# yoshitomo-matsubara/sc2-benchmark

Hardware: AMD Instinct MI355X
Metric: images/s + bpp, Entropic-Student ResNet-50 224^2 (higher is better)
Workload: dtype bf16

## Files before the change

### sc2-benchmark_amd/csrc/conv1x1_pair.hip

```cpp
#include <stdlib.h>

#include <atomic>

#include "gfx950_prims.h"

#ifndef SC2_NT_PAIR
#define SC2_NT_PAIR 0
#endif

namespace {

using namespace sc2prim;

#ifndef SC2_PAIR_DBG
#define SC2_PAIR_DBG 0
#endif

struct PairArgs {
    const uint16_t *__restrict__ o;
    const uint16_t *__restrict__ w3;
    const float *__restrict__ b3;
    const uint16_t *__restrict__ idn;
    uint16_t *__restrict__ h;
    const uint16_t *__restrict__ w1;
    const float *__restrict__ b1;
    uint16_t *__restrict__ u;
    int M, n_tiles;
    int rev;
    unsigned *tile_ctr;
};

template <int C, int K1, int N2, int MT>
__global__ __launch_bounds__(512, 2) void conv1x1_pair_kernel(const PairArgs p) {
    constexpr int P = MT * 16;
    constexpr int KS1 = K1 / 32, KS2 = C / 32;
    constexpr int NT1 = C / 8 / 16;
    constexpr int ROWB = C * 2;
    constexpr int CPR = ROWB / 16;
    constexpr int IMG = P * ROWB, SLAB = P * 64, OT = KS1 * SLAB;
    constexpr int NT2 = N2 / 128;
    static_assert(N2 == 128 || N2 == 256, "one or two 16-channel tiles of u per wave");
    static_assert(N2 <= C, "the u staging lives in the image region");
    static_assert(CPR == 64, "one image row = one LDS-DMA wave-instruction");
    constexpr int UROW = N2 * 2, UCPR = UROW / 16;
    constexpr int OQ = (P * K1 * 2 / 16 + 511) / 512;
    constexpr int UQ = (P * UCPR + 511) / 512;
    constexpr int IQ = (P * CPR + 511) / 512;
    extern __shared__ __attribute__((aligned(16))) unsigned char smem[];
    unsigned char *img = smem;
    unsigned char *ot = smem + IMG;
    volatile int *next_slot = reinterpret_cast<volatile int *>(smem + IMG + OT);
    float *bias_lds = reinterpret_cast<float *>(smem + IMG + OT + 16);

    const uint32_t lds_base = (uint32_t)(uintptr_t)(lds_ptr_t)smem;
    const int tid = threadIdx.x, lane = tid & 63;
    const int wn = __builtin_amdgcn_readfirstlane(tid >> 6);

    constexpr uint32_t OOB = 0x80000000u;
    const buf_rsrc_t rs_idn = make_rsrc(p.idn, (uint32_t)((long long)p.M * ROWB));
    const buf_rsrc_t rs_o = make_rsrc(p.o, (uint32_t)((long long)p.M * K1 * 2));
    const buf_rsrc_t rs_h = make_rsrc(p.h, (uint32_t)((long long)p.M * ROWB));
    const buf_rsrc_t rs_u = make_rsrc(p.u, (uint32_t)((long long)p.M * N2 * 2));

    auto load_o = [&](int tile, uint4 (&ov)[OQ], int tq) {
        const bool t_ok = tile < p.n_tiles;
        const int tpos = p.rev ? p.n_tiles - 1 - tile : tile;
        const uint32_t so = (uint32_t)(t_ok ? (long long)tpos * P * (K1 * 2) : 0);
#pragma unroll
        for (int k = 0; k < OQ; ++k) {
            const int q = tq + 512 * k;
            const bool ok = t_ok && q < P * (K1 / 8) && (long long)tpos * P + q / (K1 / 8) < p.M;
            ov[k] = buf_load16(rs_o, ok ? (uint32_t)q * 16u : OOB, so);
        }
    };
    auto store_o = [&](const uint4 (&ov)[OQ], int tq) {
#pragma unroll
        for (int k = 0; k < OQ; ++k) {
            const int q = tq + 512 * k;
            if (q < P * (K1 / 8)) {
                const int row = q / (K1 / 8), c16 = q % (K1 / 8);
                lds_write16(lds_base + IMG + (c16 >> 2) * SLAB + row * 64 + (((c16 & 3) ^ ((row >> 1) & 3)) << 4),
                            __builtin_bit_cast(u32x4_t, ov[k]));
            }
        }
    };
    auto issue_identity = [&](int tile, int lq) {
        static_assert(P % 8 == 0, "every wave takes P / 8 rows: straight-line issue, exact vmcnt bookkeeping");
#pragma unroll
        for (int r = 0; r < P / 8; ++r) {
            const int row = wn + 8 * r;
            const long long m = (long long)(p.rev ? p.n_tiles - 1 - tile : tile) * P + row;
            const bool ok = tile < p.n_tiles && m < p.M && !(SC2_PAIR_DBG & 1);
            const uint32_t voff = ok ? (uint32_t)((lq ^ (row & 15)) << 4) : OOB;
            buf_load_lds16(rs_idn, (lds_ptr_t)(img + row * ROWB), voff, (uint32_t)(ok ? m * ROWB : 0));
        }
    };

    uint4 wv[KS1][NT1];
    const buf_rsrc_t rs_w3 = make_rsrc(p.w3, (uint32_t)(C * K1 * 2));
    const uint32_t w3_vo = (uint32_t)(((wn * NT1) * KS1 * 64 + lane) * 16);
    auto load_w = [&]() {
#pragma unroll
        for (int j = 0; j < NT1; ++j)
#pragma unroll
            for (int s = 0; s < KS1; ++s) wv[s][j] = buf_load16(rs_w3, w3_vo, (uint32_t)((j * KS1 + s) * 1024));
    };
    load_w();
    const buf_rsrc_t rs_w1 = make_rsrc(p.w1, (uint32_t)(N2 * C * 2));
    const uint32_t w1_vo = (uint32_t)(((wn * NT2) * KS2 * 64 + lane) * 16);

    for (int k = tid; k < C + N2; k += 512) bias_lds[k] = k < C ? p.b3[k] : p.b1[k - C];
    int tile = blockIdx.x;
    int next_tile = tile + gridDim.x;
    {
        uint4 ov[OQ];
        load_o(tile, ov, tid);
        store_o(ov, tid);
        issue_identity(tile, lane);
    }
    __syncthreads();

    bool first = true;
    while (tile < p.n_tiles) {
        const long long m0 = (long long)(p.rev ? p.n_tiles - 1 - tile : tile) * P;
        int tq = tid, lq = lane;
        asm volatile("" : "+v"(tq), "+v"(lq));
        const int frow = lq & 15, fq = lq >> 4;
        const int o_lane = frow * 64 + ((fq ^ ((frow >> 1) & 3)) << 4);
        const int img_row = frow * ROWB;
        unsigned claimed = 0;
        if (tid == 0) {
            const unsigned one = 1u;
            asm volatile("global_atomic_add %0, %1, %2, off sc0" : "=v"(claimed) : "v"(p.tile_ctr), "v"(one) : "memory");
        }
        f32x4_t acc[MT][NT1];
#pragma unroll
        for (int i = 0; i < MT; ++i)
#pragma unroll
            for (int j = 0; j < NT1; ++j) acc[i][j] = f32x4_t{0.f, 0.f, 0.f, 0.f};
        {
            const uint32_t o_addr = lds_base + IMG + o_lane;
#pragma unroll
            for (int s = 0; s < KS1; ++s) {
                u32x4_t xa[4], xb[3];
                static_assert(MT == 7, "the asm waits below name 4 + 3 registers");
                xa[0] = lds_read16_imm<0 * 1024>(o_addr + s * SLAB);
                xa[1] = lds_read16_imm<1 * 1024>(o_addr + s * SLAB);
                xa[2] = lds_read16_imm<2 * 1024>(o_addr + s * SLAB);
                xa[3] = lds_read16_imm<3 * 1024>(o_addr + s * SLAB);
                asm volatile("s_waitcnt lgkmcnt(0)" : "+v"(xa[0]), "+v"(xa[1]), "+v"(xa[2]), "+v"(xa[3])::"memory");
                xb[0] = lds_read16_imm<4 * 1024>(o_addr + s * SLAB);
                xb[1] = lds_read16_imm<5 * 1024>(o_addr + s * SLAB);
                xb[2] = lds_read16_imm<6 * 1024>(o_addr + s * SLAB);
#pragma unroll
                for (int i = 0; i < 4; ++i) {
                    const bf16x8_t xf = __builtin_bit_cast(bf16x8_t, xa[i]);
#pragma unroll
                    for (int j = 0; j < NT1; ++j)
                        acc[i][j] = __builtin_amdgcn_mfma_f32_16x16x32_bf16(__builtin_bit_cast(bf16x8_t, wv[s][j]), xf, acc[i][j], 0, 0, 0);
                }
                asm volatile("s_waitcnt lgkmcnt(0)" : "+v"(xb[0]), "+v"(xb[1]), "+v"(xb[2])::"memory");
#pragma unroll
                for (int i = 0; i < 3; ++i) {
                    const bf16x8_t xf = __builtin_bit_cast(bf16x8_t, xb[i]);
#pragma unroll
                    for (int j = 0; j < NT1; ++j)
                        acc[4 + i][j] = __builtin_amdgcn_mfma_f32_16x16x32_bf16(__builtin_bit_cast(bf16x8_t, wv[s][j]), xf, acc[4 + i][j], 0, 0, 0);
                }
                __builtin_amdgcn_sched_barrier(0);
            }
        }
        if (first) asm volatile("s_waitcnt vmcnt(0)" ::: "memory");
        else if (wn == 0) asm volatile("s_waitcnt vmcnt(%0)" ::"n"(IQ + UQ + 1) : "memory");
        else asm volatile("s_waitcnt vmcnt(%0)" ::"n"(IQ + UQ) : "memory");
        first = false;
        __syncthreads();
#pragma unroll
        for (int j = 0; j < NT1; ++j) {
            const int c16 = wn * (NT1 * 2) + j * 2 + (fq >> 1);
            const float4 b3v = *reinterpret_cast<const float4 *>(bias_lds + wn * (NT1 * 16) + j * 16 + fq * 4);
            const f32x2_t b01 = {b3v.x, b3v.y}, b23 = {b3v.z, b3v.w};
            const int slot_lane = img_row + ((c16 ^ frow) << 4) + (fq & 1) * 8;
#pragma unroll
            for (int i = 0; i < MT; ++i) {
                unsigned char *slot = img + slot_lane + i * (16 * ROWB);
                const uint2 xr = *reinterpret_cast<const uint2 *>(slot);
                f32x2_t v01 = f32x2_t{acc[i][j][0], acc[i][j][1]} + b01;
                f32x2_t v23 = f32x2_t{acc[i][j][2], acc[i][j][3]} + b23;
                v01 += f32x2_t{__builtin_bit_cast(float, xr.x << 16), __builtin_bit_cast(float, xr.x & 0xFFFF0000u)};
                v23 += f32x2_t{__builtin_bit_cast(float, xr.y << 16), __builtin_bit_cast(float, xr.y & 0xFFFF0000u)};
                v01 = f32x2_t{fmaxf(v01[0], 0.f), fmaxf(v01[1], 0.f)};
                v23 = f32x2_t{fmaxf(v23[0], 0.f), fmaxf(v23[1], 0.f)};
                uint2 o2;
                o2.x = pack2(v01);
                o2.y = pack2(v23);
                *reinterpret_cast<uint2 *>(slot) = o2;
                if ((i & 3) == 3) __builtin_amdgcn_sched_barrier(0);
            }
        }
        __syncthreads();
        __builtin_amdgcn_sched_barrier(0);
        constexpr int GB = 8;
        uint4 gb[GB][NT2];
#pragma unroll
        for (int ks = 0; ks < GB; ++ks)
#pragma unroll
            for (int t = 0; t < NT2; ++t) gb[ks][t] = buf_load16(rs_w1, w1_vo, (uint32_t)((t * KS2 + ks) * 1024));
        uint4 ov[OQ];
        load_o(next_tile, ov, tq);
        f32x4_t acc2[MT][NT2];
#pragma unroll
        for (int i = 0; i < MT; ++i)
#pragma unroll
            for (int t = 0; t < NT2; ++t) acc2[i][t] = f32x4_t{0.f, 0.f, 0.f, 0.f};
#pragma unroll
        for (int ks = 0; ks < ((SC2_PAIR_DBG & 4) ? 0 : KS2); ++ks) {
            bf16x8_t gf[NT2];
#pragma unroll
            for (int t = 0; t < NT2; ++t) {
                gf[t] = __builtin_bit_cast(bf16x8_t, gb[ks % GB][t]);
                if (ks + GB < KS2) gb[ks % GB][t] = buf_load16(rs_w1, w1_vo, (uint32_t)((t * KS2 + ks + GB) * 1024));
            }
            const int rd_lane = img_row + (((ks * 4 + fq) ^ frow) << 4);
#pragma unroll
            for (int i = 0; i < MT; ++i) {
                const bf16x8_t xf = __builtin_bit_cast(bf16x8_t, *reinterpret_cast<const uint4 *>(img + rd_lane + i * (16 * ROWB)));
#pragma unroll
                for (int t = 0; t < NT2; ++t) acc2[i][t] = __builtin_amdgcn_mfma_f32_16x16x32_bf16(gf[t], xf, acc2[i][t], 0, 0, 0);
            }
            if ((ks & 1) == 1) __builtin_amdgcn_sched_barrier(0);
        }
        if (tid == 0) {
            asm volatile("s_waitcnt vmcnt(%1)" : "+v"(claimed) : "n"(OQ) : "memory");
            *next_slot = (int)(claimed + 2 * gridDim.x);
            if (claimed == (unsigned)(p.n_tiles - 1)) *p.tile_ctr = 0u;
        }
        u32x4_t hv[IQ];
#pragma unroll
        for (int k = 0; k < IQ; ++k) {
            const int q = tq + 512 * k;
            const int row = q / CPR, c = q % CPR;
            hv[k] = *reinterpret_cast<const u32x4_t *>(img + row * ROWB + ((c ^ (row & 15)) << 4));
        }
        __syncthreads();
        store_o(ov, tq);
#pragma unroll
        for (int t = 0; t < NT2; ++t) {
            const float4 b1v = *reinterpret_cast<const float4 *>(bias_lds + C + (wn * NT2 + t) * 16 + fq * 4);
            const f32x2_t b01 = {b1v.x, b1v.y}, b23 = {b1v.z, b1v.w};
            const int c16 = (wn * NT2 + t) * 2 + (fq >> 1);
            const int u_lane = frow * UROW + ((c16 ^ frow) << 4) + (fq & 1) * 8;
#pragma unroll
            for (int i = 0; i < MT; ++i) {
                f32x2_t v01 = f32x2_t{acc2[i][t][0], acc2[i][t][1]} + b01;
                f32x2_t v23 = f32x2_t{acc2[i][t][2], acc2[i][t][3]} + b23;
                v01 = f32x2_t{fmaxf(v01[0], 0.f), fmaxf(v01[1], 0.f)};
                v23 = f32x2_t{fmaxf(v23[0], 0.f), fmaxf(v23[1], 0.f)};
                uint2 o2;
                o2.x = pack2(v01);
                o2.y = pack2(v23);
                *reinterpret_cast<uint2 *>(img + u_lane + i * (16 * UROW)) = o2;
            }
        }
        asm volatile("s_waitcnt lgkmcnt(0)" ::: "memory");
        __syncthreads();
        const int tile_after_next = __builtin_amdgcn_readfirstlane(*next_slot);
        u32x4_t uv[UQ];
#pragma unroll
        for (int k = 0; k < UQ; ++k) {
            const int q = tq + 512 * k;
            const int row = q / UCPR, c = q % UCPR;
            const int qq = q < P * UCPR ? row * UROW + ((c ^ (row & 15)) << 4) : 0;
            uv[k] = *reinterpret_cast<const u32x4_t *>(img + qq);
        }
        __syncthreads();
        issue_identity(next_tile, lq);
        {
            const uint32_t so = (uint32_t)(m0 * ROWB);
#pragma unroll
            for (int k = 0; k < IQ; ++k) {
                const int q = tq + 512 * k;
                buf_store16<SC2_NT_PAIR>(rs_h, (q < P * CPR && m0 + q / CPR < p.M && !(SC2_PAIR_DBG & 2)) ? (uint32_t)q * 16u : OOB, so, hv[k]);
            }
        }
        {
            const uint32_t so = (uint32_t)(m0 * UROW);
#pragma unroll
            for (int k = 0; k < UQ; ++k) {
                const int q = tq + 512 * k;
                buf_store16<SC2_NT_PAIR>(rs_u, (q < P * UCPR && m0 + q / UCPR < p.M && !(SC2_PAIR_DBG & 2)) ? (uint32_t)q * 16u : OOB, so, uv[k]);
            }
        }
        tile = next_tile;
        next_tile = tile_after_next;
    }
}

constexpr int kRing = 256;
sc2_counter_ring g_ring;
std::atomic<unsigned> g_seq{0};

template <int C, int K1, int N2, int MT>
int launch_pair(const PairArgs &a, hipStream_t s) {
    constexpr int P = MT * 16;
    constexpr int lds = P * C * 2 + (K1 / 32) * P * 64 + 16 + (C + N2) * 4;
    static_assert(lds <= 160 * 1024, "image + o tile must fit the CU's LDS");
    static bool attr_set[SC2_MAX_DEVICES] = {};
    const int dev = sc2_device_slot();
    if (!attr_set[dev]) {
        (void)hipFuncSetAttribute(reinterpret_cast<const void *>(&conv1x1_pair_kernel<C, K1, N2, MT>),
                                  hipFuncAttributeMaxDynamicSharedMemorySize, lds);
        attr_set[dev] = true;
    }
    const int g_cus = sc2_device_cus();
    unsigned *slot = g_ring.launch_slot(s, kRing, 1, g_seq);
    if (!slot) return SC2_ERR_INTERNAL;
    PairArgs b = a;
    b.n_tiles = (a.M + P - 1) / P;
    b.tile_ctr = slot;
    {
        const int alt = sc2_pol().pair_alt;
        static std::atomic<unsigned> calls{0};
        b.rev = alt ? (int)(calls.fetch_add(1) & 1u) : 0;
    }
    const int grid = b.n_tiles < g_cus ? b.n_tiles : g_cus;
    hipLaunchKernelGGL((conv1x1_pair_kernel<C, K1, N2, MT>), dim3(grid), dim3(512), lds, s, b);
    SC2_CHECK_LAUNCH();
    return SC2_OK;
}

}

extern "C" int sc2_conv1x1_pair_supported(int K1, int C, int N2) { return (K1 == 128 && C == 512 && (N2 == 128 || N2 == 256)) ? 1 : 0; }

extern "C" int sc2_conv1x1_pair_fwd(const void *o, const void *w3_frag, const float *b3, const void *identity, void *h,
                                    const void *w1_frag, const float *b1, void *u, long long M, int K1, int C, int N2,
                                    void *stream) {
    SC2_REQUIRE(o && w3_frag && b3 && identity && h && w1_frag && b1 && u, SC2_ERR_INVALID_ARG, "conv1x1_pair: null argument");
    SC2_REQUIRE(sc2_conv1x1_pair_supported(K1, C, N2), SC2_ERR_UNSUPPORTED, "conv1x1_pair: K1 %d C %d N2 %d not supported", K1, C, N2);
    SC2_REQUIRE(M > 0 && M * C * 2 < 0x7FF00000LL, SC2_ERR_UNSUPPORTED, "conv1x1_pair: M = %lld outside the 32-bit buffer range", M);
    PairArgs a;
    a.o = static_cast<const uint16_t *>(o); a.w3 = static_cast<const uint16_t *>(w3_frag); a.b3 = b3;
    a.idn = static_cast<const uint16_t *>(identity); a.h = static_cast<uint16_t *>(h);
    a.w1 = static_cast<const uint16_t *>(w1_frag); a.b1 = b1; a.u = static_cast<uint16_t *>(u);
    a.M = (int)M; a.n_tiles = 0; a.tile_ctr = nullptr; a.rev = 0;
    if (N2 == 256) return launch_pair<512, 128, 256, 7>(a, static_cast<hipStream_t>(stream));
    return launch_pair<512, 128, 128, 7>(a, static_cast<hipStream_t>(stream));
}
```

Baseline: 45720.

## Add double-buffered identity image pair kernel with register-resident W1 for N2=128

Adds a second fused conv1x1 pair kernel that keeps two image buffers in LDS, so the identity tile for the tile after next streams in while the current tile is computed. W1 is held in registers beside W3, which removes the per-tile W1 reloads, and the row tile shrinks from 7 to 3 MMA row tiles. The N2=128 path now dispatches to this kernel by default. It also adds optional memtime stamp instrumentation behind a compile flag. Smaller tiles mean more tiles and more atomic claims, and register pressure rises.

```diff
diff --git a/sc2-benchmark_amd/csrc/conv1x1_pair.hip b/sc2-benchmark_amd/csrc/conv1x1_pair.hip
--- a/sc2-benchmark_amd/csrc/conv1x1_pair.hip
+++ b/sc2-benchmark_amd/csrc/conv1x1_pair.hip
@@ -14,6 +14,33 @@
 
 #ifndef SC2_PAIR_DBG
 #define SC2_PAIR_DBG 0
+#endif
+
+#ifndef SC2_PAIR_STAMPS
+#define SC2_PAIR_STAMPS 0
+#endif
+constexpr int N_STAMP = 12;
+#if SC2_PAIR_STAMPS
+#include <stdio.h>
+#define PAIR_STAMPS_BEGIN unsigned long long st_sum[N_STAMP] = {}, st_last = __builtin_amdgcn_s_memtime(); const unsigned long long st_first = st_last
+#define PAIR_STAMP(k)                                                   \
+    do {                                                                \
+        __builtin_amdgcn_sched_barrier(0);                              \
+        const unsigned long long t_ = __builtin_amdgcn_s_memtime();     \
+        st_sum[k] += t_ - st_last;                                      \
+        st_last = t_;                                                   \
+        __builtin_amdgcn_sched_barrier(0);                              \
+    } while (0)
+#define PAIR_STAMPS_END                                                                                        \
+    do {                                                                                                       \
+        st_sum[10] = st_last - st_first;                                                                       \
+        if (p.stamps && lane == 0)                                                                             \
+            for (int k = 0; k < N_STAMP; ++k) p.stamps[((size_t)blockIdx.x * 8 + wn) * N_STAMP + k] = st_sum[k]; \
+    } while (0)
+#else
+#define PAIR_STAMPS_BEGIN do {} while (0)
+#define PAIR_STAMP(k) do {} while (0)
+#define PAIR_STAMPS_END do {} while (0)
 #endif
 
 struct PairArgs {
@@ -28,6 +55,9 @@
     int M, n_tiles;
     int rev;
     unsigned *tile_ctr;
+#if SC2_PAIR_STAMPS
+    unsigned long long *stamps;
+#endif
 };
 
 template <int C, int K1, int N2, int MT>
@@ -121,6 +151,7 @@
     __syncthreads();
 
     bool first = true;
+    PAIR_STAMPS_BEGIN;
     while (tile < p.n_tiles) {
         const long long m0 = (long long)(p.rev ? p.n_tiles - 1 - tile : tile) * P;
         int tq = tid, lq = lane;
@@ -170,11 +201,14 @@
                 __builtin_amdgcn_sched_barrier(0);
             }
         }
+        PAIR_STAMP(0);
         if (first) asm volatile("s_waitcnt vmcnt(0)" ::: "memory");
         else if (wn == 0) asm volatile("s_waitcnt vmcnt(%0)" ::"n"(IQ + UQ + 1) : "memory");
         else asm volatile("s_waitcnt vmcnt(%0)" ::"n"(IQ + UQ) : "memory");
         first = false;
+        PAIR_STAMP(1);
         __syncthreads();
+        PAIR_STAMP(2);
 #pragma unroll
         for (int j = 0; j < NT1; ++j) {
             const int c16 = wn * (NT1 * 2) + j * 2 + (fq >> 1);
@@ -199,6 +233,7 @@
             }
         }
         __syncthreads();
+        PAIR_STAMP(3);
         __builtin_amdgcn_sched_barrier(0);
         constexpr int GB = 8;
         uint4 gb[GB][NT2];
@@ -230,6 +265,7 @@
             }
             if ((ks & 1) == 1) __builtin_amdgcn_sched_barrier(0);
         }
+        PAIR_STAMP(4);
         if (tid == 0) {
             asm volatile("s_waitcnt vmcnt(%1)" : "+v"(claimed) : "n"(OQ) : "memory");
             *next_slot = (int)(claimed + 2 * gridDim.x);
@@ -243,6 +279,7 @@
             hv[k] = *reinterpret_cast<const u32x4_t *>(img + row * ROWB + ((c ^ (row & 15)) << 4));
         }
         __syncthreads();
+        PAIR_STAMP(5);
         store_o(ov, tq);
 #pragma unroll
         for (int t = 0; t < NT2; ++t) {
@@ -264,6 +301,7 @@
         }
         asm volatile("s_waitcnt lgkmcnt(0)" ::: "memory");
         __syncthreads();
+        PAIR_STAMP(6);
         const int tile_after_next = __builtin_amdgcn_readfirstlane(*next_slot);
         u32x4_t uv[UQ];
 #pragma unroll
@@ -274,6 +312,7 @@
             uv[k] = *reinterpret_cast<const u32x4_t *>(img + qq);
         }
         __syncthreads();
+        PAIR_STAMP(7);
         issue_identity(next_tile, lq);
         {
             const uint32_t so = (uint32_t)(m0 * ROWB);
@@ -293,7 +332,341 @@
         }
         tile = next_tile;
         next_tile = tile_after_next;
-    }
+        PAIR_STAMP(8);
+#if SC2_PAIR_STAMPS
+        st_sum[11] += 1;
+#endif
+    }
+    PAIR_STAMPS_END;
+}
+
+template <int OFF>
+__device__ __forceinline__ u32x2_t lds_read8_imm(uint32_t addr) {
+    u32x2_t v;
+    asm volatile("ds_read_b64 %0, %1 offset:%2" : "=v"(v) : "v"(addr), "n"(OFF) : "memory");
+    return v;
+}
+template <int OFF>
+__device__ __forceinline__ void lds_write8_imm(uint32_t addr, u32x2_t v) {
+    asm volatile("ds_write_b64 %0, %1 offset:%2" ::"v"(addr), "v"(v), "n"(OFF) : "memory");
+}
+__device__ __forceinline__ void wg_barrier() { asm volatile("s_waitcnt lgkmcnt(0)\n\ts_barrier" ::: "memory"); }
+
+template <int C, int K1, int N2, int MT>
+__global__ __launch_bounds__(512, 2) void conv1x1_pair_2img_kernel(const PairArgs p) {
+    constexpr int P = MT * 16;
+    constexpr int KS1 = K1 / 32, KS2 = C / 32;
+    constexpr int NT1 = C / 8 / 16;
+    constexpr int ROWB = C * 2;
+    constexpr int CPR = ROWB / 16;
+    constexpr int OQ = (P * K1 * 2 / 16 + 511) / 512;
+    constexpr int PO = OQ * 512 / (K1 / 8);
+    static_assert(PO >= P && OQ * 512 % (K1 / 8) == 0, "whole padded rows");
+    constexpr int IMG = P * ROWB, SLAB = PO * 64, OT = KS1 * SLAB;
+    constexpr int NT2 = N2 / 128;
+    static_assert(NT2 == 1, "W1 resident in registers beside W3 (64 + 64); N2 = 256 would take 128 and stays on the kernel above");
+    static_assert(N2 <= C, "the u staging lives in the image region");
+    static_assert(CPR == 64, "one image row = one LDS-DMA wave-instruction");
+    static_assert(P % 8 == 0, "every wave takes P / 8 identity rows: straight-line issue, exact vmcnt bookkeeping");
+    static_assert((MT - 1) * 16 * ROWB < 65536, "row tiles are reached through the 16-bit offset field");
+    constexpr int UROW = N2 * 2, UCPR = UROW / 16;
+    constexpr int UQ = (P * UCPR + 511) / 512;
+    constexpr int IQ = (P * CPR + 511) / 512;
+    static_assert(P * CPR == IQ * 512, "every thread reads IQ whole chunks of the image");
+    constexpr int SLOT = 2 * IMG + OT, BIAS = SLOT + 16;
+    extern __shared__ __attribute__((aligned(16))) unsigned char smem[];
+
+    const uint32_t lds_base = (uint32_t)(uintptr_t)(lds_ptr_t)smem;
+    const int tid = threadIdx.x, lane = tid & 63;
+    const int wn = __builtin_amdgcn_readfirstlane(tid >> 6);
+
+    constexpr uint32_t OOB = 0x80000000u;
+    const buf_rsrc_t rs_idn = make_rsrc(p.idn, (uint32_t)((long long)p.M * ROWB));
+    const buf_rsrc_t rs_o = make_rsrc(p.o, (uint32_t)((long long)p.M * K1 * 2));
+    const buf_rsrc_t rs_h = make_rsrc(p.h, (uint32_t)((long long)p.M * ROWB));
+    const buf_rsrc_t rs_u = make_rsrc(p.u, (uint32_t)((long long)p.M * N2 * 2));
+
+    auto load_o = [&](int tile, uint4 (&ov)[OQ], int tq) {
+        const bool t_ok = tile < p.n_tiles;
+        const int tpos = p.rev ? p.n_tiles - 1 - tile : tile;
+        const uint32_t so = (uint32_t)(t_ok ? (long long)tpos * P * (K1 * 2) : 0);
+#pragma unroll
+        for (int k = 0; k < OQ; ++k) {
+            const int q = tq + 512 * k;
+            const bool ok = t_ok && q < P * (K1 / 8) && (long long)tpos * P + q / (K1 / 8) < p.M;
+            ov[k] = buf_load16(rs_o, ok ? (uint32_t)q * 16u : OOB, so);
+        }
+    };
+    auto store_o = [&](const uint4 (&ov)[OQ], int tq) {
+#pragma unroll
+        for (int k = 0; k < OQ; ++k) {
+            const int q = tq + 512 * k;
+            const int row = q / (K1 / 8), c16 = q % (K1 / 8);
+            lds_write16(lds_base + 2 * IMG + (c16 >> 2) * SLAB + row * 64 + (((c16 & 3) ^ ((row >> 1) & 3)) << 4),
+                        __builtin_bit_cast(u32x4_t, ov[k]));
+        }
+    };
+    auto issue_identity = [&](int tile, uint32_t buf, int lq) {
+#pragma unroll
+        for (int r = 0; r < P / 8; ++r) {
+            const int row = wn + 8 * r;
+            const long long m = (long long)(p.rev ? p.n_tiles - 1 - tile : tile) * P + row;
+            const bool ok = tile < p.n_tiles && m < p.M && !(SC2_PAIR_DBG & 1);
+            const uint32_t voff = ok ? (uint32_t)((lq ^ (row & 15)) << 4) : OOB;
+            buf_load_lds16(rs_idn, (lds_ptr_t)(smem + buf + row * ROWB), voff, (uint32_t)(ok ? m * ROWB : 0));
+        }
+    };
+
+    {
+        float *bias_lds = reinterpret_cast<float *>(smem + BIAS);
+        for (int k = tid; k < C + N2; k += 512) bias_lds[k] = k < C ? p.b3[k] : p.b1[k - C];
+    }
+    int tile = blockIdx.x;
+    int next_tile = tile + gridDim.x;
+    issue_identity(tile, 0, lane);
+    issue_identity(next_tile, IMG, lane);
+    u32x4_t wv[KS1][NT1];
+    const buf_rsrc_t rs_w3 = make_rsrc(p.w3, (uint32_t)(C * K1 * 2));
+    const uint32_t w3_vo = (uint32_t)(((wn * NT1) * KS1 * 64 + lane) * 16);
+#pragma unroll
+    for (int j = 0; j < NT1; ++j)
+#pragma unroll
+        for (int s = 0; s < KS1; ++s) wv[s][j] = __builtin_bit_cast(u32x4_t, buf_load16(rs_w3, w3_vo, (uint32_t)((j * KS1 + s) * 1024)));
+    const buf_rsrc_t rs_w1 = make_rsrc(p.w1, (uint32_t)(N2 * C * 2));
+    const uint32_t w1_vo = (uint32_t)(((wn * NT2) * KS2 * 64 + lane) * 16);
+    u32x4_t w1v[KS2];
+#pragma unroll
+    for (int ks = 0; ks < KS2; ++ks) w1v[ks] = __builtin_bit_cast(u32x4_t, buf_load16(rs_w1, w1_vo, (uint32_t)(ks * 1024)));
+    {
+        uint4 ov[OQ];
+        load_o(tile, ov, tid);
+        store_o(ov, tid);
+    }
+#pragma unroll
+    for (int j = 0; j < NT1; ++j)
+#pragma unroll
+        for (int s = 0; s < KS1; ++s) asm volatile("" : "+v"(wv[s][j]));
+#pragma unroll
+    for (int ks = 0; ks < KS2; ++ks) asm volatile("" : "+v"(w1v[ks]));
+    asm volatile("s_waitcnt vmcnt(0)" ::: "memory");
+    wg_barrier();
+
+    uint32_t cur = 0;
+    PAIR_STAMPS_BEGIN;
+    while (tile < p.n_tiles) {
+        const long long m0 = (long long)(p.rev ? p.n_tiles - 1 - tile : tile) * P;
+        int tq = tid, lq = lane;
+        asm volatile("" : "+v"(tq), "+v"(lq));
+        const int frow = lq & 15, fq = lq >> 4;
+        const uint32_t o_addr = lds_base + 2 * IMG + frow * 64 + ((fq ^ ((frow >> 1) & 3)) << 4);
+        const uint32_t img_cur = lds_base + cur;
+        const uint32_t img_row = img_cur + frow * ROWB;
+        unsigned claimed = 0;
+        if (tid == 0) {
+            const unsigned one = 1u;
+            asm volatile("global_atomic_add %0, %1, %2, off sc0" : "=v"(claimed) : "v"(p.tile_ctr), "v"(one) : "memory");
+        }
+        f32x4_t acc[MT][NT1];
+#pragma unroll
+        for (int i = 0; i < MT; ++i)
+#pragma unroll
+            for (int j = 0; j < NT1; ++j) acc[i][j] = f32x4_t{0.f, 0.f, 0.f, 0.f};
+        static_assert(MT == 3, "the asm waits below name three registers per k-step");
+        {
+            u32x4_t x[2][MT];
+            x[0][0] = lds_read16_imm<0 * 1024>(o_addr);
+            x[0][1] = lds_read16_imm<1 * 1024>(o_addr);
+            x[0][2] = lds_read16_imm<2 * 1024>(o_addr);
+#pragma unroll
+            for (int s = 0; s < KS1; ++s) {
+                u32x4_t(&xc)[MT] = x[s & 1];
+                if (s + 1 < KS1) {
+                    u32x4_t(&xn)[MT] = x[(s + 1) & 1];
+                    xn[0] = lds_read16_imm<0 * 1024>(o_addr + (s + 1) * SLAB);
+                    xn[1] = lds_read16_imm<1 * 1024>(o_addr + (s + 1) * SLAB);
+                    xn[2] = lds_read16_imm<2 * 1024>(o_addr + (s + 1) * SLAB);
+                    asm volatile("s_waitcnt lgkmcnt(%3)" : "+v"(xc[0]), "+v"(xc[1]), "+v"(xc[2]) : "n"(MT) : "memory");
+                } else {
+                    asm volatile("s_waitcnt lgkmcnt(0)" : "+v"(xc[0]), "+v"(xc[1]), "+v"(xc[2])::"memory");
+                }
+#pragma unroll
+                for (int i = 0; i < MT; ++i) {
+                    const bf16x8_t xf = __builtin_bit_cast(bf16x8_t, xc[i]);
+#pragma unroll
+                    for (int j = 0; j < NT1; ++j)
+                        acc[i][j] = __builtin_amdgcn_mfma_f32_16x16x32_bf16(__builtin_bit_cast(bf16x8_t, wv[s][j]), xf, acc[i][j], 0, 0, 0);
+                }
+                __builtin_amdgcn_sched_barrier(0);
+            }
+        }
+        PAIR_STAMP(0);
+        u32x4_t b3r[NT1];
+#pragma unroll
+        for (int j = 0; j < NT1; ++j) b3r[j] = lds_read16_imm<0>(lds_base + (uint32_t)(BIAS + (wn * (NT1 * 16) + j * 16 + fq * 4) * 4));
+        if (wn == 0) asm volatile("s_waitcnt vmcnt(%0)" ::"n"(P / 8 + IQ + UQ + 1) : "memory");
+        else asm volatile("s_waitcnt vmcnt(%0)" ::"n"(P / 8 + IQ + UQ) : "memory");
+        PAIR_STAMP(1);
+        wg_barrier();
+        PAIR_STAMP(2);
+        {
+            u32x2_t xr[NT1][MT];
+            uint32_t slot[NT1];
+#pragma unroll
+            for (int j = 0; j < NT1; ++j) {
+                const int c16 = wn * (NT1 * 2) + j * 2 + (fq >> 1);
+                slot[j] = img_row + ((c16 ^ frow) << 4) + (fq & 1) * 8;
+                xr[j][0] = lds_read8_imm<0 * 16 * ROWB>(slot[j]);
+                xr[j][1] = lds_read8_imm<1 * 16 * ROWB>(slot[j]);
+                xr[j][2] = lds_read8_imm<2 * 16 * ROWB>(slot[j]);
+            }
+#pragma unroll
+            for (int j = 0; j < NT1; ++j) {
+                asm volatile("s_waitcnt lgkmcnt(%4)" : "+v"(xr[j][0]), "+v"(xr[j][1]), "+v"(xr[j][2]), "+v"(b3r[j]) : "n"(MT * (NT1 - 1)) : "memory");
+                const f32x4_t b3v = __builtin_bit_cast(f32x4_t, b3r[j]);
+                const f32x2_t b01 = {b3v[0], b3v[1]}, b23 = {b3v[2], b3v[3]};
+                u32x2_t o2[MT];
+#pragma unroll
+                for (int i = 0; i < MT; ++i) {
+                    f32x2_t v01 = f32x2_t{acc[i][j][0], acc[i][j][1]} + b01;
+                    f32x2_t v23 = f32x2_t{acc[i][j][2], acc[i][j][3]} + b23;
+                    v01 += f32x2_t{bf_lo(xr[j][i][0]), bf_hi(xr[j][i][0])};
+                    v23 += f32x2_t{bf_lo(xr[j][i][1]), bf_hi(xr[j][i][1])};
+                    v01 = f32x2_t{fmaxf(v01[0], 0.f), fmaxf(v01[1], 0.f)};
+                    v23 = f32x2_t{fmaxf(v23[0], 0.f), fmaxf(v23[1], 0.f)};
+                    o2[i] = u32x2_t{pack2(v01), pack2(v23)};
+                }
+                lds_write8_imm<0 * 16 * ROWB>(slot[j], o2[0]);
+                lds_write8_imm<1 * 16 * ROWB>(slot[j], o2[1]);
+                lds_write8_imm<2 * 16 * ROWB>(slot[j], o2[2]);
+            }
+        }
+        wg_barrier();
+        PAIR_STAMP(3);
+        __builtin_amdgcn_sched_barrier(0);
+        uint4 ov[OQ];
+        load_o(next_tile, ov, tq);
+        f32x4_t acc2[MT][NT2];
+#pragma unroll
+        for (int i = 0; i < MT; ++i)
+#pragma unroll
+            for (int t = 0; t < NT2; ++t) acc2[i][t] = f32x4_t{0.f, 0.f, 0.f, 0.f};
+        {
+            constexpr int KS2E = (SC2_PAIR_DBG & 4) ? 0 : KS2;
+            u32x4_t x[2][MT];
+            {
+                const uint32_t a = img_row + ((fq ^ frow) << 4);
+                x[0][0] = lds_read16_imm<0 * 16 * ROWB>(a);
+                x[0][1] = lds_read16_imm<1 * 16 * ROWB>(a);
+                x[0][2] = lds_read16_imm<2 * 16 * ROWB>(a);
+            }
+#pragma unroll
+            for (int ks = 0; ks < KS2E; ++ks) {
+                u32x4_t(&xc)[MT] = x[ks & 1];
+                if (ks + 1 < KS2E) {
+                    u32x4_t(&xn)[MT] = x[(ks + 1) & 1];
+                    const uint32_t a = img_row + ((((ks + 1) * 4 + fq) ^ frow) << 4);
+                    xn[0] = lds_read16_imm<0 * 16 * ROWB>(a);
+                    xn[1] = lds_read16_imm<1 * 16 * ROWB>(a);
+                    xn[2] = lds_read16_imm<2 * 16 * ROWB>(a);
+                    asm volatile("s_waitcnt lgkmcnt(%3)" : "+v"(xc[0]), "+v"(xc[1]), "+v"(xc[2]) : "n"(MT) : "memory");
+                } else {
+                    asm volatile("s_waitcnt lgkmcnt(0)" : "+v"(xc[0]), "+v"(xc[1]), "+v"(xc[2])::"memory");
+                }
+                const bf16x8_t gf = __builtin_bit_cast(bf16x8_t, w1v[ks]);
+#pragma unroll
+                for (int i = 0; i < MT; ++i)
+                    acc2[i][0] = __builtin_amdgcn_mfma_f32_16x16x32_bf16(gf, __builtin_bit_cast(bf16x8_t, xc[i]), acc2[i][0], 0, 0, 0);
+                if ((ks & 1) == 1) __builtin_amdgcn_sched_barrier(0);
+            }
+            if (KS2E == 0) asm volatile("s_waitcnt lgkmcnt(0)" : "+v"(x[0][0]), "+v"(x[0][1]), "+v"(x[0][2])::"memory");
+        }
+        PAIR_STAMP(4);
+        if (tid == 0) {
+            asm volatile("s_waitcnt vmcnt(%1)" : "+v"(claimed) : "n"(OQ) : "memory");
+            const unsigned nxt = claimed + 2 * gridDim.x;
+            asm volatile("ds_write_b32 %0, %1" ::"v"(lds_base + (uint32_t)SLOT), "v"(nxt) : "memory");
+            if (claimed == (unsigned)(p.n_tiles - 1)) *p.tile_ctr = 0u;
+        }
+        u32x4_t hv[IQ];
+#pragma unroll
+        for (int k = 0; k < IQ; ++k) {
+            const int q = tq + 512 * k;
+            const int row = q / CPR, c = q % CPR;
+            hv[k] = __builtin_bit_cast(u32x4_t, lds_read16(img_cur + row * ROWB + ((c ^ (row & 15)) << 4)));
+        }
+        static_assert(IQ == 6, "the wait below names six registers");
+        asm volatile("s_waitcnt lgkmcnt(0)" : "+v"(hv[0]), "+v"(hv[1]), "+v"(hv[2]), "+v"(hv[3]), "+v"(hv[4]), "+v"(hv[5])::"memory");
+        wg_barrier();
+        PAIR_STAMP(5);
+        store_o(ov, tq);
+        {
+            u32x4_t b1r[NT2];
+#pragma unroll
+            for (int t = 0; t < NT2; ++t) b1r[t] = lds_read16_imm<0>(lds_base + (uint32_t)(BIAS + C * 4 + ((wn * NT2 + t) * 16 + fq * 4) * 4));
+            asm volatile("s_waitcnt lgkmcnt(0)" : "+v"(b1r[0])::"memory");
+#pragma unroll
+            for (int t = 0; t < NT2; ++t) {
+                const f32x4_t b1v = __builtin_bit_cast(f32x4_t, b1r[t]);
+                const f32x2_t b01 = {b1v[0], b1v[1]}, b23 = {b1v[2], b1v[3]};
+                const int c16 = (wn * NT2 + t) * 2 + (fq >> 1);
+                const uint32_t u_lane = img_cur + frow * UROW + ((c16 ^ frow) << 4) + (fq & 1) * 8;
+                u32x2_t o2[MT];
+#pragma unroll
+                for (int i = 0; i < MT; ++i) {
+                    f32x2_t v01 = f32x2_t{acc2[i][t][0], acc2[i][t][1]} + b01;
+                    f32x2_t v23 = f32x2_t{acc2[i][t][2], acc2[i][t][3]} + b23;
+                    v01 = f32x2_t{fmaxf(v01[0], 0.f), fmaxf(v01[1], 0.f)};
+                    v23 = f32x2_t{fmaxf(v23[0], 0.f), fmaxf(v23[1], 0.f)};
+                    o2[i] = u32x2_t{pack2(v01), pack2(v23)};
+                }
+                lds_write8_imm<0 * 16 * UROW>(u_lane, o2[0]);
+                lds_write8_imm<1 * 16 * UROW>(u_lane, o2[1]);
+                lds_write8_imm<2 * 16 * UROW>(u_lane, o2[2]);
+            }
+        }
+        wg_barrier();
+        PAIR_STAMP(6);
+        unsigned slot_v;
+        asm volatile("ds_read_b32 %0, %1" : "=v"(slot_v) : "v"(lds_base + (uint32_t)SLOT) : "memory");
+        u32x4_t uv[UQ];
+#pragma unroll
+        for (int k = 0; k < UQ; ++k) {
+            const int q = tq + 512 * k;
+            const int row = q / UCPR, c = q % UCPR;
+            const int qq = q < P * UCPR ? row * UROW + ((c ^ (row & 15)) << 4) : 0;
+            uv[k] = __builtin_bit_cast(u32x4_t, lds_read16(img_cur + qq));
+        }
+        static_assert(UQ == 2, "the wait below names two registers");
+        asm volatile("s_waitcnt lgkmcnt(0)" : "+v"(slot_v), "+v"(uv[0]), "+v"(uv[1])::"memory");
+        const int tile_after_next = __builtin_amdgcn_readfirstlane((int)slot_v);
+        wg_barrier();
+        PAIR_STAMP(7);
+        issue_identity(tile_after_next, cur, lq);
+        {
+            const uint32_t so = (uint32_t)(m0 * ROWB);
+#pragma unroll
+            for (int k = 0; k < IQ; ++k) {
+                const int q = tq + 512 * k;
+                buf_store16<SC2_NT_PAIR>(rs_h, (m0 + q / CPR < p.M && !(SC2_PAIR_DBG & 2)) ? (uint32_t)q * 16u : OOB, so, hv[k]);
+            }
+        }
+        {
+            const uint32_t so = (uint32_t)(m0 * UROW);
+#pragma unroll
+            for (int k = 0; k < UQ; ++k) {
+                const int q = tq + 512 * k;
+                buf_store16<SC2_NT_PAIR>(rs_u, (q < P * UCPR && m0 + q / UCPR < p.M && !(SC2_PAIR_DBG & 2)) ? (uint32_t)q * 16u : OOB, so, uv[k]);
+            }
+        }
+        tile = next_tile;
+        next_tile = tile_after_next;
+        cur ^= (uint32_t)IMG;
+        PAIR_STAMP(8);
+#if SC2_PAIR_STAMPS
+        st_sum[11] += 1;
+#endif
+    }
+    PAIR_STAMPS_END;
 }
 
 constexpr int kRing = 256;
@@ -303,13 +676,17 @@
 template <int C, int K1, int N2, int MT>
 int launch_pair(const PairArgs &a, hipStream_t s) {
     constexpr int P = MT * 16;
-    constexpr int lds = P * C * 2 + (K1 / 32) * P * 64 + 16 + (C + N2) * 4;
-    static_assert(lds <= 160 * 1024, "image + o tile must fit the CU's LDS");
+    constexpr bool TWO = MT == 3;
+    constexpr int PO = TWO ? (P * (K1 / 8) + 511) / 512 * 512 / (K1 / 8) : P;
+    constexpr int lds = (TWO ? 2 : 1) * P * C * 2 + (K1 / 32) * PO * 64 + 16 + (C + N2) * 4;
+    static_assert(lds <= 160 * 1024, "images + o tile must fit the CU's LDS");
+    const void *kern;
+    if constexpr (TWO) kern = reinterpret_cast<const void *>(&conv1x1_pair_2img_kernel<C, K1, N2, MT>);
+    else kern = reinterpret_cast<const void *>(&conv1x1_pair_kernel<C, K1, N2, MT>);
     static bool attr_set[SC2_MAX_DEVICES] = {};
     const int dev = sc2_device_slot();
     if (!attr_set[dev]) {
-        (void)hipFuncSetAttribute(reinterpret_cast<const void *>(&conv1x1_pair_kernel<C, K1, N2, MT>),
-                                  hipFuncAttributeMaxDynamicSharedMemorySize, lds);
+        (void)hipFuncSetAttribute(kern, hipFuncAttributeMaxDynamicSharedMemorySize, lds);
         attr_set[dev] = true;
     }
     const int g_cus = sc2_device_cus();
@@ -324,7 +701,30 @@
         b.rev = alt ? (int)(calls.fetch_add(1) & 1u) : 0;
     }
     const int grid = b.n_tiles < g_cus ? b.n_tiles : g_cus;
-    hipLaunchKernelGGL((conv1x1_pair_kernel<C, K1, N2, MT>), dim3(grid), dim3(512), lds, s, b);
+#if SC2_PAIR_STAMPS
+    const char *stamp_path = getenv("SC2_PAIR_STAMPS");
+    const size_t stamp_bytes = (size_t)grid * 8 * N_STAMP * sizeof(unsigned long long);
+    b.stamps = nullptr;
+    if (stamp_path) {
+        void *sp = nullptr;
+        (void)hipMalloc(&sp, stamp_bytes);
+        (void)hipMemset(sp, 0, stamp_bytes);
+        b.stamps = static_cast<unsigned long long *>(sp);
+    }
+#endif
+    if constexpr (TWO) hipLaunchKernelGGL((conv1x1_pair_2img_kernel<C, K1, N2, MT>), dim3(grid), dim3(512), lds, s, b);
+    else hipLaunchKernelGGL((conv1x1_pair_kernel<C, K1, N2, MT>), dim3(grid), dim3(512), lds, s, b);
+#if SC2_PAIR_STAMPS
+    if (b.stamps) {
+        (void)hipStreamSynchronize(s);
+        unsigned long long *host = static_cast<unsigned long long *>(malloc(stamp_bytes));
+        (void)hipMemcpy(host, b.stamps, stamp_bytes, hipMemcpyDeviceToHost);
+        (void)hipFree(b.stamps);
+        FILE *f = fopen(stamp_path, "wb");
+        if (f) { fwrite(host, 1, stamp_bytes, f); fclose(f); }
+        free(host);
+    }
+#endif
     SC2_CHECK_LAUNCH();
     return SC2_OK;
 }
@@ -345,5 +745,8 @@
     a.w1 = static_cast<const uint16_t *>(w1_frag); a.b1 = b1; a.u = static_cast<uint16_t *>(u);
     a.M = (int)M; a.n_tiles = 0; a.tile_ctr = nullptr; a.rev = 0;
     if (N2 == 256) return launch_pair<512, 128, 256, 7>(a, static_cast<hipStream_t>(stream));
+#if SC2_PAIR_STAMPS == 2
     return launch_pair<512, 128, 128, 7>(a, static_cast<hipStream_t>(stream));
+#endif
+    return launch_pair<512, 128, 128, 3>(a, static_cast<hipStream_t>(stream));
 }
```

After: 46070, median of 6. No clear change (+0.7%).
